# cbalint13/opencv-dlco

Measured on AMD Instinct MI355X. Metric: pj-learn patch-pairs/sec, higher is better.
Workload: dtype f32; 1 GPU; pj-learn configs[1] Liberty-shaped, rank ~64: 500000 pair-rows x PR-dim 8192, batch 200+200 per GPU (global 200+200), mu=0.0025 gamma=0.5, fp32, rank 48 after 3893 steps; device= (gfx950:sramecc+:xnack-), burn_in_steps=300

## Files before the change

opencv-dlco_amd/csrc/kernels_bf16x2.hip:

```cpp
#include "dlco_internal.hpp"
#include "split_bf16_dev.hpp"

#include <algorithm>

namespace dlco {

namespace {

constexpr int W8 = 8;
constexpr int T8 = 64 * W8;
constexpr int KS = 4;

__global__ __launch_bounds__(256) void split_x_kernel(const float *X, long ldx, int M, int MT, int K, bf16x8 *hi, bf16x8 *lo,
                                                      bf16x8 *lo2)
{
    const long t = (long)blockIdx.x * blockDim.x + threadIdx.x;
    const long total = (long)(K / 16) * MT * 64;
    if (t >= total) return;
    const int lane = (int)(t & 63);
    const long q = t >> 6;
    const int tile = (int)(q % MT);
    const int k16 = (int)(q / MT);
    const int row = tile * 32 + (lane & 31), k = k16 * 16 + 8 * (lane >> 5);
    bf16x8 h, l, l2;
    if (row < M) {
        const f32x4 a = *reinterpret_cast<const f32x4 *>(X + (long)row * ldx + k);
        const f32x4 b = *reinterpret_cast<const f32x4 *>(X + (long)row * ldx + k + 4);
#pragma unroll
        for (int j = 0; j < 8; j++) split_f32<3>(j < 4 ? a[j & 3] : b[j & 3], j, h, l, l2);
    } else {
        h = l = l2 = bf16x8{};
    }
    hi[t] = h;
    lo[t] = l;
    if (lo2) lo2[t] = l2;
}

struct Bf2Dev {
    int M, N, K;
    const bf16x8 *xhi, *xlo, *xlo2;
    const float *G;
    long ldg;
    float *slab;
    int tiled;
};

template <int MT, int NS>
__global__ __launch_bounds__(T8) void skinny_bf16x2_kernel(Bf2Dev g)
{
    __shared__ float red[4 * MT * 16 * 64];
    const int lane = threadIdx.x & 63, wave = threadIdx.x >> 6;
    const int lc = lane & 31, lh = lane >> 5;
    const int ct = wave & 3, kh = wave >> 2;
    const int col = blockIdx.x * 128 + ct * 32 + lc;
    const int nsteps = g.K / 16;
    const int per = nsteps / ((int)gridDim.y * 2);
    const int s0 = (blockIdx.y * 2 + kh) * per, s1 = s0 + per;

    f32x16 acc[MT];
#pragma unroll
    for (int a = 0; a < MT; a++)
#pragma unroll
        for (int r = 0; r < 16; r++) acc[a][r] = 0.f;

    bf16x8 ah[MT], al[MT], ahn[MT], aln[MT];
    bf16x8 am[NS == 3 ? MT : 1], amn[NS == 3 ? MT : 1];
    auto load_g = [&](int s, float (&gv)[8]) {
        const float *p = g.G + ((long)s * 16 + 8 * lh) * g.ldg + col;
#pragma unroll
        for (int j = 0; j < 8; j++) gv[j] = p[(long)j * g.ldg];
    };
    auto load_a = [&](int s, bf16x8 (&h)[MT], bf16x8 (&l)[MT], bf16x8 (&m2)[NS == 3 ? MT : 1]) {
#pragma unroll
        for (int t = 0; t < MT; t++) {
            const long idx = plane_entry((long)s, MT, t, lane);
            h[t] = g.xhi[idx];
            l[t] = g.xlo[idx];
            if (NS == 3) m2[t] = g.xlo2[idx];
        }
    };
    auto compute = [&](const float (&gv)[8], const bf16x8 (&h)[MT], const bf16x8 (&l)[MT], const bf16x8 (&m2)[NS == 3 ? MT : 1]) {
        bf16x8 bh, bl, bl2;
        split_frag<NS>(gv, bh, bl, bl2);
        mfma_split_terms<MT, NS>(h, l, m2, bh, bl, bl2, acc);
    };

    float gq[4][8];
    const int last = s1 - 1;
#pragma unroll
    for (int q = 0; q < 4; q++) load_g(s0 + q, gq[q]);
    load_a(s0, ah, al, am);
    load_a(s0 + 1, ahn, aln, amn);
    for (int s = s0; s < s1; s += 4) {
        compute(gq[0], ah, al, am);
        load_g(min(s + 4, last), gq[0]);
        load_a(min(s + 2, last), ah, al, am);
        compute(gq[1], ahn, aln, amn);
        load_g(min(s + 5, last), gq[1]);
        load_a(min(s + 3, last), ahn, aln, amn);
        compute(gq[2], ah, al, am);
        load_g(min(s + 6, last), gq[2]);
        load_a(min(s + 4, last), ah, al, am);
        compute(gq[3], ahn, aln, amn);
        load_g(min(s + 7, last), gq[3]);
        load_a(min(s + 5, last), ahn, aln, amn);
    }

    if (kh == 1) {
#pragma unroll
        for (int a = 0; a < MT; a++)
#pragma unroll
            for (int r = 0; r < 16; r++) red[((ct * MT + a) * 16 + r) * 64 + lane] = acc[a][r];
    }
    __syncthreads();
    if (kh == 0) {
        float *slab = g.slab + (long)blockIdx.y * g.M * g.N;
#pragma unroll
        for (int a = 0; a < MT; a++)
#pragma unroll
            for (int r = 0; r < 16; r++) {
                const float s = acc[a][r] + red[((ct * MT + a) * 16 + r) * 64 + lane];
                const int i = a * 32 + (r & 3) + 8 * (r >> 2) + 4 * lh;
                if (i < g.M) slab[(long)i * g.N + col] = s;
            }
    }
}


template <int MT, int NS>
__global__ __launch_bounds__(SB_T) void skinny_rows_kernel(Bf2Dev g)
{
    extern __shared__ __attribute__((aligned(16))) char lds_raw[];
    constexpr int ABYTES = sb_abytes(MT, NS);
    constexpr int APLANE = MT * 256;
    constexpr int NA = NS * MT;
    float *gb0 = reinterpret_cast<float *>(lds_raw), *gb1 = reinterpret_cast<float *>(lds_raw + SB_GBYTES);
    bf16x8 *ab0 = reinterpret_cast<bf16x8 *>(lds_raw + 2 * SB_GBYTES), *ab1 = reinterpret_cast<bf16x8 *>(lds_raw + 2 * SB_GBYTES + ABYTES);
    const int tid = threadIdx.x, lane = tid & 63, wave = tid >> 6;
    int bx = blockIdx.x, by = blockIdx.y;
    {
        const int gx = gridDim.x, ks = gridDim.y;
        if (ks <= 8 && 8 % ks == 0 && (gx * ks) % 8 == 0 && gx % (8 / ks) == 0) {
            const int b = by * gx + bx, xcd = b & 7, w = b >> 3, per = 8 / ks;
            by = xcd / per;
            bx = w * per + xcd % per;
        }
    }
    const int j0 = bx * 128;
    const int kslice = g.K / (int)gridDim.y;
    const int kbeg = by * kslice;
    const int nchunks = kslice / SB_KC;
    const int st0 = kbeg / 16;

    if (wave >= 8) {
        const int lt = tid - 512, grow = lt >> 4, gc4 = lt & 15;
        const __amdgpu_buffer_rsrc_t rsrc =
            __builtin_amdgcn_make_buffer_rsrc(const_cast<float *>(g.G), 0, (int)((long)g.K * g.ldg * (long)sizeof(float)), 0x00020000);
        const long pitch = g.tiled ? 128 : g.ldg;
        const long base = g.tiled ? ((long)bx * (g.K / 128) + kbeg / 128) * 16384 + (long)grow * 128 + 4 * gc4
                                  : (long)(j0 + grow) * g.ldg + kbeg + 4 * gc4;
        const int voff = (int)(base * (long)sizeof(float));
        const int row16 = (int)(16 * pitch * (long)sizeof(float));
        const PlaneRsrc rs = make_plane_rsrc<MT, NS>(g.xhi, g.xlo, g.xlo2, g.K);
        struct Stage { f32x4 gq[8]; bf16x8 aq[NA]; };
        Stage s0, s1;
        auto gload = [&](int c, Stage &st) {
            const int soff = g.tiled ? ((c >> 1) * 16384 + (c & 1) * 64) * (int)sizeof(float) : c * SB_KC * (int)sizeof(float);
#pragma unroll
            for (int u = 0; u < 8; u++) st.gq[u] = __builtin_bit_cast(f32x4, __builtin_amdgcn_raw_buffer_load_b128(rsrc, voff, soff + u * row16, 0));
            const int a0 = slice_bytes<MT>(st0 + 4 * c);
#pragma unroll
            for (int v = 0; v < NA; v++) st.aq[v] = load_slice_entry<MT>(rs, a0, lt, v);
        };
        auto gstore = [&](int buf, const Stage &st) {
            float *gb = buf ? gb1 : gb0;
            bf16x8 *ab = buf ? ab1 : ab0;
#pragma unroll
            for (int u = 0; u < 8; u++) *reinterpret_cast<f32x4 *>(gb + (grow + 16 * u) * SB_RS + 4 * gc4) = st.gq[u];
#pragma unroll
            for (int v = 0; v < NA; v++) ab[lt + 256 * v] = st.aq[v];
        };
        const int last = nchunks - 1;
        gload(0, s0);
        gload(min(1, last), s1);
        gstore(0, s0);
        gload(min(2, last), s0);
        __syncthreads();
        auto full = [&](int buf, Stage &set, int cc) { gstore(buf, set); gload(cc + 3, set); __syncthreads(); };
        auto part = [&](int buf, Stage &set, int cc) {
            if (cc >= nchunks) return;
            if (cc + 1 < nchunks) gstore(buf, set);
            if (cc + 3 < nchunks) gload(cc + 3, set);
            __syncthreads();
        };
        int c = 0;
        for (; c + 4 < nchunks; c += 2) { full(1, s1, c); full(0, s0, c + 1); }
        part(1, s1, c); part(0, s0, c + 1); part(1, s1, c + 2); part(0, s0, c + 3);
        __syncthreads();
        return;
    }

    const int lc = lane & 31, lh = lane >> 5;
    const int nt = wave & 3, kh = wave >> 2;
    f32x16 acc[MT];
#pragma unroll
    for (int a = 0; a < MT; a++)
#pragma unroll
        for (int r = 0; r < 16; r++) acc[a][r] = 0.f;

    auto fetch = [&](const float *gb, const bf16x8 *ab, int q, Frag<MT, NS> &f) {
        const float *p = gb + (nt * 32 + lc) * SB_RS + 16 * q + 8 * lh;
        f.g0 = *reinterpret_cast<const f32x4 *>(p);
        f.g1 = *reinterpret_cast<const f32x4 *>(p + 4);
#pragma unroll
        for (int n = 0; n < NS; n++)
#pragma unroll
            for (int t = 0; t < MT; t++) f.a[n][t] = ab[n * APLANE + plane_entry(q, MT, t, lane)];
    };
    auto multiply = [&](const Frag<MT, NS> &f) {
        bf16x8 bh, bl, bl2;
        split_frag<NS>(f.g0, f.g1, bh, bl, bl2);
        mfma_split_terms<MT, NS>(f.a[0], f.a[NS >= 2 ? 1 : 0], f.a[NS - 1], bh, bl, bl2, acc);
    };
    Frag<MT, NS> fa;
    __syncthreads();
    for (int c = 0; c < nchunks; c++) {
        const float *gb = (c & 1) ? gb1 : gb0;
        const bf16x8 *ab = (c & 1) ? ab1 : ab0;
        fetch(gb, ab, 2 * kh, fa);
        multiply(fa);
        fetch(gb, ab, 2 * kh + 1, fa);
        multiply(fa);
        __syncthreads();
    }

    float *red = reinterpret_cast<float *>(lds_raw);
    if (kh == 1) {
#pragma unroll
        for (int a = 0; a < MT; a++)
#pragma unroll
            for (int r = 0; r < 16; r++) red[((nt * MT + a) * 16 + r) * 64 + lane] = acc[a][r];
    }
    __syncthreads();
    if (kh == 0) {
        float *slab = g.slab + (long)by * g.M * g.N;
        const int col = j0 + nt * 32 + lc;
#pragma unroll
        for (int a = 0; a < MT; a++)
#pragma unroll
            for (int r = 0; r < 16; r++) {
                const float sum = acc[a][r] + red[((nt * MT + a) * 16 + r) * 64 + lane];
                const int i = a * 32 + (r & 3) + 8 * (r >> 2) + 4 * lh;
                if (i < g.M) slab[(long)i * g.N + col] = sum;
            }
    }
}

__global__ __launch_bounds__(256) void reduce_split_kernel(const float *slab, int split, int M, int MT, int N, float *C, long ldc, float alpha,
                                                           const float *E1, float b1, const float *E2, float b2, bf16x8 *hi, bf16x8 *lo)
{
    const long total = (long)M * N, q = N >> 3;
    for (long e = (long)blockIdx.x * blockDim.x + threadIdx.x; e < (long)M * q; e += (long)gridDim.x * blockDim.x) {
        const int i = (int)(e / q), k8 = (int)(e % q), j = k8 * 8;
        const float *p = slab + (long)i * N + j;
        f32x4 s0 = *reinterpret_cast<const f32x4 *>(p), s1 = *reinterpret_cast<const f32x4 *>(p + 4);
        for (int z = 1; z < split; z++) {
            s0 += *reinterpret_cast<const f32x4 *>(p + (long)z * total);
            s1 += *reinterpret_cast<const f32x4 *>(p + (long)z * total + 4);
        }
        const long idx = (long)i * ldc + j;
        f32x4 o0 = alpha * s0, o1 = alpha * s1;
        if (E1) { o0 += b1 * *reinterpret_cast<const f32x4 *>(E1 + idx); o1 += b1 * *reinterpret_cast<const f32x4 *>(E1 + idx + 4); }
        if (E2) { o0 += b2 * *reinterpret_cast<const f32x4 *>(E2 + idx); o1 += b2 * *reinterpret_cast<const f32x4 *>(E2 + idx + 4); }
        *reinterpret_cast<f32x4 *>(C + idx) = o0;
        *reinterpret_cast<f32x4 *>(C + idx + 4) = o1;
        bf16x8 h, l, l2;
        split_frag<2>(o0, o1, h, l, l2);
        const long t = plane_entry_at(MT, i, k8);
        hi[t] = h;
        lo[t] = l;
    }
}

constexpr int SYM_TS = 132;
static_assert(SB_KC * SYM_TS * 4 <= SB_GBYTES, "a transposed chunk image must fit the G image");

struct SymDev {
    int M, K;
    int nt, lb;
    const bf16x8 *xhi, *xlo, *xlo2;
    const float *G;
    float *slab;
};

template <int MT, int NS, bool FULL>
__global__ __launch_bounds__(SB_T) void skinny_sym_kernel(SymDev g)
{
    extern __shared__ __attribute__((aligned(16))) char lds_raw[];
    constexpr int ABYTES = sb_abytes(MT, NS);
    constexpr int APLANE = MT * 256;
    constexpr int NA = NS * MT;
    const int NT = g.nt, lb = g.lb;
    float *gb0 = reinterpret_cast<float *>(lds_raw), *gb1 = reinterpret_cast<float *>(lds_raw + SB_GBYTES);
    bf16x8 *ab0 = reinterpret_cast<bf16x8 *>(lds_raw + 2 * SB_GBYTES), *ab1 = reinterpret_cast<bf16x8 *>(lds_raw + 2 * SB_GBYTES + ABYTES);
    __shared__ int jlist[16];
    const int tid = threadIdx.x, lane = tid & 63, wave = tid >> 6;
    const int xcd = blockIdx.x & 7, slot = blockIdx.x >> 3;
    const int p = xcd >> 1, c = xcd & 1;
    int I;
    if (p == 0 || p == 3) I = (c << (lb - 1)) | slot;
    else {
        const int b5 = slot >> (lb - 2), b4 = p == 1 ? c : (b5 ^ c);
        I = (b5 << (lb - 1)) | (b4 << (lb - 2)) | (slot & ((1 << (lb - 2)) - 1));
    }
    if (I >= NT) return;
    const int dbase = (p == 0 ? 1 : (p == 1 ? 2 : (p == 2 ? 3 : 0))) << (lb - 2);
    int nchunks;
    if (FULL) nchunks = 2 << (lb - 2);
    else {
        const int nslots = 1 << (lb - 2);
        int cnt = 0;
        for (int sl = 0; sl < nslots; sl++) {
            const int J = I ^ (dbase | sl);
            if (J < NT) { if (tid == 0) jlist[cnt] = J; cnt++; }
        }
        nchunks = 2 * cnt;
        __syncthreads();
    }
    if (!FULL && nchunks == 0) {
        float *slab = g.slab + (long)p * g.M * g.K;
        for (int e = tid; e < g.M * 128; e += SB_T) slab[(long)(e >> 7) * g.K + I * 128 + (e & 127)] = 0.f;
        return;
    }
    auto partner = [&](int cc) { return FULL ? (I ^ (dbase | (cc >> 1))) : jlist[cc >> 1]; };
    auto tile_bytes = [&](int J) {
        const int a = min(I, J), b = max(I, J);
        return (a * NT - a * (a - 1) / 2 + (b - a)) * (128 * 128 * (int)sizeof(float));
    };

    if (wave >= 8) {
        const int lt = tid - 512;
        const int voff_d = ((lt >> 4) * 128 + 4 * (lt & 15)) * (int)sizeof(float);
        const int voff_t = ((lt >> 5) * 128 + 4 * (lt & 31)) * (int)sizeof(float);
        const int loff_d = (lt >> 4) * SB_RS + 4 * (lt & 15), loff_t = (lt >> 5) * SYM_TS + 4 * (lt & 31);
        const __amdgpu_buffer_rsrc_t rsrc =
            __builtin_amdgcn_make_buffer_rsrc(const_cast<float *>(g.G), 0, (NT * (NT + 1) / 2) * 128 * 128 * (int)sizeof(float), 0x00020000);
        const PlaneRsrc rs = make_plane_rsrc<MT, NS>(g.xhi, g.xlo, g.xlo2, g.K);
        struct Stage { f32x4 gq[8]; bf16x8 aq[NA]; };
        Stage s0, s1;
        auto gload = [&](int cc, Stage &st) {
            const int J = __builtin_amdgcn_readfirstlane(partner(cc)), half = cc & 1;
            const bool direct = I <= J;
            const int voff = direct ? voff_d : voff_t;
            const int soff = tile_bytes(J) + (direct ? half * 64 : half * 64 * 128) * (int)sizeof(float);
            const int ustep = (direct ? 16 : 8) * 128 * (int)sizeof(float);
            const int a0 = slice_bytes<MT>(J * 8 + half * 4);
            __builtin_amdgcn_sched_barrier(0);
#pragma unroll
            for (int u = 0; u < 8; u++) {
                st.gq[u] = __builtin_bit_cast(f32x4, __builtin_amdgcn_raw_buffer_load_b128(rsrc, voff, soff + u * ustep, 0));
                __builtin_amdgcn_sched_barrier(0);
            }
#pragma unroll
            for (int v = 0; v < NA; v++) {
                st.aq[v] = load_slice_entry<MT>(rs, a0, lt, v);
                __builtin_amdgcn_sched_barrier(0);
            }
        };
        auto gstore = [&](int cc, const Stage &st) {
            float *gb = (cc & 1) ? gb1 : gb0;
            bf16x8 *ab = (cc & 1) ? ab1 : ab0;
            const bool direct = I <= partner(cc);
            const int loff = direct ? loff_d : loff_t, lstep = direct ? 16 * SB_RS : 8 * SYM_TS;
#pragma unroll
            for (int u = 0; u < 8; u++) *reinterpret_cast<f32x4 *>(gb + loff + u * lstep) = st.gq[u];
#pragma unroll
            for (int v = 0; v < NA; v++) ab[lt + 256 * v] = st.aq[v];
        };
        gload(0, s0);
        gload(1, s1);
        gstore(0, s0);
        gload(min(2, nchunks - 1), s0);
        __syncthreads();
        int cc = 0;
        for (; cc + 4 < nchunks; cc += 2) {
            gstore(cc + 1, s1); gload(cc + 3, s1); __syncthreads();
            gstore(cc + 2, s0); gload(cc + 4, s0); __syncthreads();
        }
        for (; cc < nchunks; cc += 2) {
            if (cc + 1 < nchunks) gstore(cc + 1, s1);
            if (cc + 3 < nchunks) gload(cc + 3, s1);
            __syncthreads();
            if (cc + 2 < nchunks) gstore(cc + 2, s0);
            if (cc + 4 < nchunks) gload(cc + 4, s0);
            __syncthreads();
        }
        __syncthreads();
        return;
    }

    const int lc = lane & 31, lh = lane >> 5;
    const int nt = wave & 3, kh = wave >> 2;
    f32x16 acc[MT];
#pragma unroll
    for (int a = 0; a < MT; a++)
#pragma unroll
        for (int r = 0; r < 16; r++) acc[a][r] = 0.f;

    auto fetch = [&](const float *gb, const bf16x8 *ab, bool direct, int q, Frag<MT, NS> &f) {
        if (direct) {
            const float *pp = gb + (nt * 32 + lc) * SB_RS + 16 * q + 8 * lh;
            f.g0 = *reinterpret_cast<const f32x4 *>(pp);
            f.g1 = *reinterpret_cast<const f32x4 *>(pp + 4);
        } else {
            const float *pp = gb + (16 * q + 8 * lh) * SYM_TS + nt * 32 + lc;
#pragma unroll
            for (int j = 0; j < 4; j++) { f.g0[j] = pp[j * SYM_TS]; f.g1[j] = pp[(4 + j) * SYM_TS]; }
        }
#pragma unroll
        for (int n = 0; n < NS; n++)
#pragma unroll
            for (int t = 0; t < MT; t++) f.a[n][t] = ab[n * APLANE + plane_entry(q, MT, t, lane)];
    };
    auto multiply = [&](const Frag<MT, NS> &f) {
        bf16x8 bh, bl, bl2;
        split_frag<NS>(f.g0, f.g1, bh, bl, bl2);
        mfma_split_terms<MT, NS>(f.a[0], f.a[NS >= 2 ? 1 : 0], f.a[NS - 1], bh, bl, bl2, acc);
    };
    Frag<MT, NS> fa;
    __syncthreads();
    for (int cc = 0; cc < nchunks; cc++) {
        const float *gb = (cc & 1) ? gb1 : gb0;
        const bf16x8 *ab = (cc & 1) ? ab1 : ab0;
        const bool direct = I <= partner(cc);
        fetch(gb, ab, direct, 2 * kh, fa);
        multiply(fa);
        fetch(gb, ab, direct, 2 * kh + 1, fa);
        multiply(fa);
        __syncthreads();
    }

    float *red = reinterpret_cast<float *>(lds_raw);
    if (kh == 1) {
#pragma unroll
        for (int a = 0; a < MT; a++)
#pragma unroll
            for (int r = 0; r < 16; r++) red[((nt * MT + a) * 16 + r) * 64 + lane] = acc[a][r];
    }
    __syncthreads();
    if (kh == 0) {
        float *slab = g.slab + (long)p * g.M * g.K;
        const int col = I * 128 + nt * 32 + lc;
#pragma unroll
        for (int a = 0; a < MT; a++)
#pragma unroll
            for (int r = 0; r < 16; r++) {
                const float sum = acc[a][r] + red[((nt * MT + a) * 16 + r) * 64 + lane];
                const int i = a * 32 + (r & 3) + 8 * (r >> 2) + 4 * lh;
                if (i < g.M) slab[(long)i * g.K + col] = sum;
            }
    }
}

template <int MT, int NS>
void launch_sym(const SymDev &g, hipStream_t s)
{
    const size_t lds = sb_lds_bytes(MT, NS);
    if (g.nt == (1 << g.lb)) {
        ensure_dynamic_lds(reinterpret_cast<const void *>(skinny_sym_kernel<MT, NS, true>), (int)lds);
        hipLaunchKernelGGL((skinny_sym_kernel<MT, NS, true>), dim3(4u << g.lb), dim3(SB_T), lds, s, g);
    } else {
        ensure_dynamic_lds(reinterpret_cast<const void *>(skinny_sym_kernel<MT, NS, false>), (int)lds);
        hipLaunchKernelGGL((skinny_sym_kernel<MT, NS, false>), dim3(4u << g.lb), dim3(SB_T), lds, s, g);
    }
}

template <int MT, int NS>
void launch_rows(const Bf2Dev &g, dim3 grid, hipStream_t s)
{
    const size_t lds = sb_lds_bytes(MT, NS);
    ensure_dynamic_lds(reinterpret_cast<const void *>(skinny_rows_kernel<MT, NS>), (int)lds);
    hipLaunchKernelGGL((skinny_rows_kernel<MT, NS>), grid, dim3(SB_T), lds, s, g);
}

}

void split_planes_bf16(const float *X, long ldx, int M, int K, void *hi, void *lo, void *lo2, hipStream_t s)
{
    const int mt = (M + 31) / 32;
    const long total = (long)(K / 16) * mt * 64;
    hipLaunchKernelGGL(split_x_kernel, dim3((unsigned)((total + 255) / 256)), dim3(256), 0, s, X, ldx, M, mt, K,
                       static_cast<bf16x8 *>(hi), static_cast<bf16x8 *>(lo), static_cast<bf16x8 *>(lo2));
    DLCO_HIP(hipGetLastError());
}

size_t bf16x2_plane_bytes(int M, int K) { return (size_t)((M + 31) / 32) * 32 * K * sizeof(__bf16); }
size_t bf16x2_slab_floats(int M, int N, int ksplit) { return (size_t)(ksplit > 0 ? ksplit : KS) * M * N; }

bool skinny_product_bf16x2(const float *X, long ldx, int M, const float *G, long ldg, int N, int K, float alpha, float *C,
                           long ldc, const float *E1, float b1, const float *E2, float b2, void *plane_hi, void *plane_lo,
                           float *slab, hipStream_t s, int ksplit, void *plane_lo2, bool g_tiled)
{
    const int mt = (M + 31) / 32;
    const int ks = ksplit > 0 ? ksplit : KS;
    if (M < 1 || mt > 5 || N % 128 != 0 || K % (16 * ks * 2 * 4) != 0) return false;
    if (ldx % 4 != 0 || (reinterpret_cast<uintptr_t>(X) & 15) != 0) return false;
    split_planes_bf16(X, ldx, M, K, plane_hi, plane_lo, plane_lo2, s);
    Bf2Dev g;
    g.M = M; g.N = N; g.K = K;
    g.xhi = static_cast<const bf16x8 *>(plane_hi); g.xlo = static_cast<const bf16x8 *>(plane_lo);
    g.xlo2 = static_cast<const bf16x8 *>(plane_lo2);
    g.G = G; g.ldg = ldg; g.slab = slab; g.tiled = g_tiled ? 1 : 0;
    const dim3 grid(N / 128, ks), block(T8);
    if (N == K && K % (128 * ks) == 0 && ldg % 4 == 0 && (reinterpret_cast<uintptr_t>(G) & 15) == 0 &&
        (long)K * ldg * 4 < (1L << 31) && !(mt >= 4 && plane_lo2)) {
        if (plane_lo2) dispatch_mt<4>(mt, [&](auto MT) { launch_rows<MT(), 3>(g, grid, s); });
        else dispatch_mt<5>(mt, [&](auto MT) { launch_rows<MT(), 2>(g, grid, s); });
        DLCO_HIP(hipGetLastError());
        splitk_reduce_f32(slab, ks, M, N, C, ldc, alpha, 0.f, E1, b1, E2, b2, s);
        return true;
    }
    if (g_tiled || mt > 4) return false;
    if (plane_lo2) dispatch_mt<4>(mt, [&](auto MT) { hipLaunchKernelGGL((skinny_bf16x2_kernel<MT(), 3>), grid, block, 0, s, g); });
    else dispatch_mt<4>(mt, [&](auto MT) { hipLaunchKernelGGL((skinny_bf16x2_kernel<MT(), 2>), grid, block, 0, s, g); });
    DLCO_HIP(hipGetLastError());
    splitk_reduce_f32(slab, ks, M, N, C, ldc, alpha, 0.f, E1, b1, E2, b2, s);
    return true;
}

bool skinny_product_sym(const float *X, long ldx, int M, const float *Gpacked, int F, float alpha, float *C, long ldc,
                        const float *E1, float b1, const float *E2, float b2, void *plane_hi, void *plane_lo, float *slab,
                        hipStream_t s, void *plane_lo2, bool planes_ready, bool emit_planes)
{
    const int mt = (M + 31) / 32;
    const int nt = F / 128;
    if (F % 128 != 0 || nt < 1 || nt > 64 || M < 1 || mt > 5 || (mt >= 4 && plane_lo2)) return false;
    if (ldx % 4 != 0 || (reinterpret_cast<uintptr_t>(X) & 15) != 0 || (reinterpret_cast<uintptr_t>(Gpacked) & 15) != 0) return false;
    if ((planes_ready || emit_planes) && plane_lo2) return false;
    if (!planes_ready) split_planes_bf16(X, ldx, M, F, plane_hi, plane_lo, plane_lo2, s);
    SymDev g;
    g.M = M; g.K = F;
    g.nt = nt; g.lb = 2;
    while ((1 << g.lb) < nt) g.lb++;
    g.xhi = static_cast<const bf16x8 *>(plane_hi); g.xlo = static_cast<const bf16x8 *>(plane_lo); g.xlo2 = static_cast<const bf16x8 *>(plane_lo2);
    g.G = Gpacked; g.slab = slab;
    if (plane_lo2) dispatch_mt<3>(mt, [&](auto MT) { launch_sym<MT(), 3>(g, s); });
    else dispatch_mt<5>(mt, [&](auto MT) { launch_sym<MT(), 2>(g, s); });
    DLCO_HIP(hipGetLastError());
    if (emit_planes && ldc % 4 == 0 && (reinterpret_cast<uintptr_t>(C) & 15) == 0) {
        const long work = (long)M * (F / 8);
        hipLaunchKernelGGL(reduce_split_kernel, dim3((unsigned)std::min<long>((work + 255) / 256, 4096)), dim3(256), 0, s, slab, 4, M, mt, F, C, ldc,
                           alpha, E1, b1, E2, b2, static_cast<bf16x8 *>(plane_hi), static_cast<bf16x8 *>(plane_lo));
        DLCO_HIP(hipGetLastError());
    } else {
        splitk_reduce_f32(slab, 4, M, F, C, ldc, alpha, 0.f, E1, b1, E2, b2, s);
    }
    return true;
}

}
```

Measured before the change: 710,900 pair-rows/s.

## Stream symmetric-kernel operands into a four-stage LDS ring via direct global-to-LDS loads

Replaces the producer waves' register-staged double buffer in the symmetric skinny GEMM with a four-stage LDS ring. Producers fill it with global_load_lds (buffer loads go straight into LDS) and pace themselves with explicit vmcnt waits and barriers. Consumers now use a software-pipelined loop that fetches and converts the next stage while running MFMAs on the current one, and the tile and plane layouts are re-indexed to match the new LDS image. The goal is to cut the register round-trip and LDS store work on the producers and to hide load latency, at the cost of more LDS use and fragile hand-counted waits and barriers.

```diff
diff --git a/opencv-dlco_amd/csrc/kernels_bf16x2.hip b/opencv-dlco_amd/csrc/kernels_bf16x2.hip
--- a/opencv-dlco_amd/csrc/kernels_bf16x2.hip
+++ b/opencv-dlco_amd/csrc/kernels_bf16x2.hip
@@ -2,6 +2,7 @@
 #include "split_bf16_dev.hpp"
 
 #include <algorithm>
+#include <type_traits>
 
 namespace dlco {
 
@@ -282,8 +283,20 @@
     }
 }
 
-constexpr int SYM_TS = 132;
-static_assert(SB_KC * SYM_TS * 4 <= SB_GBYTES, "a transposed chunk image must fit the G image");
+constexpr int SYM_NSTAGE = 4;
+constexpr int SYM_GBYTES = SB_ROWS * (SB_KC / 2) * 4;
+__host__ __device__ constexpr int sym_abytes(int mt, int ns) { return 2 * ns * mt * 1024; }
+__host__ __device__ constexpr int sym_stage_bytes(int mt, int ns) { return SYM_GBYTES + sym_abytes(mt, ns); }
+inline size_t sym_lds_bytes(int mt, int ns) { return (size_t)SYM_NSTAGE * sym_stage_bytes(mt, ns); }
+#ifndef SYM_PREFETCH
+#define SYM_PREFETCH 1
+#endif
+#ifndef SYM_PREFETCH_MAX
+#define SYM_PREFETCH_MAX 9
+#endif
+constexpr int SYM_LDS_MAX = 160 * 1024 - 64;
+static_assert(SYM_NSTAGE * sym_stage_bytes(5, 2) <= SYM_LDS_MAX && SYM_NSTAGE * sym_stage_bytes(3, 3) <= SYM_LDS_MAX,
+              "the ring of the largest instantiations (five row tiles two-way, three three-way) must fit the LDS");
 
 struct SymDev {
     int M, K;
@@ -293,16 +306,24 @@
     float *slab;
 };
 
+template <int N>
+__device__ __forceinline__ void wait_vmcnt()
+{
+    asm volatile("s_waitcnt vmcnt(%0)" ::"n"(N) : "memory");
+}
+
 template <int MT, int NS, bool FULL>
 __global__ __launch_bounds__(SB_T) void skinny_sym_kernel(SymDev g)
 {
     extern __shared__ __attribute__((aligned(16))) char lds_raw[];
-    constexpr int ABYTES = sb_abytes(MT, NS);
-    constexpr int APLANE = MT * 256;
-    constexpr int NA = NS * MT;
+    constexpr int STAGE = sym_stage_bytes(MT, NS);
+    constexpr int NAP = 2 * NS * MT;
+    constexpr int NPIECE = 16 + NAP;
+    constexpr int PW = (NPIECE + 3) / 4;
+    constexpr bool PF = SYM_PREFETCH && MT * NS <= SYM_PREFETCH_MAX;
+    static_assert(3 * PW <= 63, "the in-flight count must fit the vmcnt field");
+    static_assert(4 * MT * 16 * 64 * 4 <= SYM_NSTAGE * STAGE, "the K-half exchange reuses the ring");
     const int NT = g.nt, lb = g.lb;
-    float *gb0 = reinterpret_cast<float *>(lds_raw), *gb1 = reinterpret_cast<float *>(lds_raw + SB_GBYTES);
-    bf16x8 *ab0 = reinterpret_cast<bf16x8 *>(lds_raw + 2 * SB_GBYTES), *ab1 = reinterpret_cast<bf16x8 *>(lds_raw + 2 * SB_GBYTES + ABYTES);
     __shared__ int jlist[16];
     const int tid = threadIdx.x, lane = tid & 63, wave = tid >> 6;
     const int xcd = blockIdx.x & 7, slot = blockIdx.x >> 3;
@@ -315,87 +336,92 @@
     }
     if (I >= NT) return;
     const int dbase = (p == 0 ? 1 : (p == 1 ? 2 : (p == 2 ? 3 : 0))) << (lb - 2);
-    int nchunks;
-    if (FULL) nchunks = 2 << (lb - 2);
+    int nst;
+    unsigned jmask = 0;
+    if (FULL) nst = 4 << (lb - 2);
     else {
         const int nslots = 1 << (lb - 2);
         int cnt = 0;
         for (int sl = 0; sl < nslots; sl++) {
             const int J = I ^ (dbase | sl);
-            if (J < NT) { if (tid == 0) jlist[cnt] = J; cnt++; }
-        }
-        nchunks = 2 * cnt;
+            if (J < NT) { if (tid == 0) jlist[cnt] = J; cnt++; jmask |= 1u << sl; }
+        }
+        nst = 4 * cnt;
         __syncthreads();
     }
-    if (!FULL && nchunks == 0) {
+    if (!FULL && nst == 0) {
         float *slab = g.slab + (long)p * g.M * g.K;
         for (int e = tid; e < g.M * 128; e += SB_T) slab[(long)(e >> 7) * g.K + I * 128 + (e & 127)] = 0.f;
         return;
     }
-    auto partner = [&](int cc) { return FULL ? (I ^ (dbase | (cc >> 1))) : jlist[cc >> 1]; };
     auto tile_bytes = [&](int J) {
         const int a = min(I, J), b = max(I, J);
         return (a * NT - a * (a - 1) / 2 + (b - a)) * (128 * 128 * (int)sizeof(float));
     };
 
     if (wave >= 8) {
-        const int lt = tid - 512;
-        const int voff_d = ((lt >> 4) * 128 + 4 * (lt & 15)) * (int)sizeof(float);
-        const int voff_t = ((lt >> 5) * 128 + 4 * (lt & 31)) * (int)sizeof(float);
-        const int loff_d = (lt >> 4) * SB_RS + 4 * (lt & 15), loff_t = (lt >> 5) * SYM_TS + 4 * (lt & 31);
-        const __amdgpu_buffer_rsrc_t rsrc =
-            __builtin_amdgcn_make_buffer_rsrc(const_cast<float *>(g.G), 0, (NT * (NT + 1) / 2) * 128 * 128 * (int)sizeof(float), 0x00020000);
-        const PlaneRsrc rs = make_plane_rsrc<MT, NS>(g.xhi, g.xlo, g.xlo2, g.K);
-        struct Stage { f32x4 gq[8]; bf16x8 aq[NA]; };
-        Stage s0, s1;
-        auto gload = [&](int cc, Stage &st) {
-            const int J = __builtin_amdgcn_readfirstlane(partner(cc)), half = cc & 1;
+        const int lw = __builtin_amdgcn_readfirstlane(wave - 8);
+        const char *Gb = reinterpret_cast<const char *>(g.G);
+        const int off_d = (lane & 15) * 512 + (lane >> 4) * 16;
+        const int off_t0 = (lane >> 5) * 512 + (lane & 31) * 16, off_t1 = (lane >> 5) * 512 + ((lane & 31) ^ 8) * 16;
+        const char *asrc[PW - 4];
+        int adst[PW - 4];
+#pragma unroll
+        for (int i = 4; i < PW; i++) {
+            const int a = min(lw + 4 * i - 16, NAP - 1);
+            const int akh = a / (NS * MT), part = (a / MT) % NS, t = a % MT;
+            const bf16x8 *plane = part == 0 ? g.xhi : (part == 1 ? g.xlo : g.xlo2);
+            asrc[i - 4] = reinterpret_cast<const char *>(plane) + (2 * akh * MT + t) * 1024 + lane * 16;
+            adst[i - 4] = SYM_GBYTES + a * 1024;
+        }
+        int J = 0;
+        auto issue = [&](int st) {
+            if ((st & 3) == 0) {
+                if (FULL) J = I ^ (dbase | (st >> 2));
+                else {
+                    J = I ^ (dbase | (__builtin_ctz(jmask)));
+                    jmask &= jmask - 1;
+                }
+                J = __builtin_amdgcn_readfirstlane(J);
+            }
+            const int half = (st >> 1) & 1, h = st & 1;
             const bool direct = I <= J;
-            const int voff = direct ? voff_d : voff_t;
-            const int soff = tile_bytes(J) + (direct ? half * 64 : half * 64 * 128) * (int)sizeof(float);
-            const int ustep = (direct ? 16 : 8) * 128 * (int)sizeof(float);
-            const int a0 = slice_bytes<MT>(J * 8 + half * 4);
-            __builtin_amdgcn_sched_barrier(0);
-#pragma unroll
-            for (int u = 0; u < 8; u++) {
-                st.gq[u] = __builtin_bit_cast(f32x4, __builtin_amdgcn_raw_buffer_load_b128(rsrc, voff, soff + u * ustep, 0));
-                __builtin_amdgcn_sched_barrier(0);
+            const char *tile = Gb + tile_bytes(J);
+            char *dst = lds_raw + (st & (SYM_NSTAGE - 1)) * STAGE;
+#pragma unroll
+            for (int i = 0; i < 4; i++) {
+                const int pc = lw + 4 * i;
+                const int od = ((pc >> 1) * 16) * 512 + half * 256 + (2 * (pc & 1) + h) * 64;
+                const int ot = (half * 64 + (2 * (i >> 1) + h) * 16 + 2 * lw + 8 * (i & 1)) * 512;
+                const int off = direct ? od + off_d : ot + ((i & 1) ? off_t1 : off_t0);
+                __builtin_amdgcn_global_load_lds((const __attribute__((address_space(1))) void *)(tile + off),
+                                                 (__attribute__((address_space(3))) void *)(dst + pc * 1024), 16, 0, 0);
             }
-#pragma unroll
-            for (int v = 0; v < NA; v++) {
-                st.aq[v] = load_slice_entry<MT>(rs, a0, lt, v);
-                __builtin_amdgcn_sched_barrier(0);
-            }
+            const int a_off = (J * 8 + half * 4 + h) * MT * 1024;
+#pragma unroll
+            for (int i = 4; i < PW; i++)
+                __builtin_amdgcn_global_load_lds((const __attribute__((address_space(1))) void *)(asrc[i - 4] + a_off),
+                                                 (__attribute__((address_space(3))) void *)(dst + adst[i - 4]), 16, 0, 0);
         };
-        auto gstore = [&](int cc, const Stage &st) {
-            float *gb = (cc & 1) ? gb1 : gb0;
-            bf16x8 *ab = (cc & 1) ? ab1 : ab0;
-            const bool direct = I <= partner(cc);
-            const int loff = direct ? loff_d : loff_t, lstep = direct ? 16 * SB_RS : 8 * SYM_TS;
-#pragma unroll
-            for (int u = 0; u < 8; u++) *reinterpret_cast<f32x4 *>(gb + loff + u * lstep) = st.gq[u];
-#pragma unroll
-            for (int v = 0; v < NA; v++) ab[lt + 256 * v] = st.aq[v];
-        };
-        gload(0, s0);
-        gload(1, s1);
-        gstore(0, s0);
-        gload(min(2, nchunks - 1), s0);
-        __syncthreads();
-        int cc = 0;
-        for (; cc + 4 < nchunks; cc += 2) {
-            gstore(cc + 1, s1); gload(cc + 3, s1); __syncthreads();
-            gstore(cc + 2, s0); gload(cc + 4, s0); __syncthreads();
-        }
-        for (; cc < nchunks; cc += 2) {
-            if (cc + 1 < nchunks) gstore(cc + 1, s1);
-            if (cc + 3 < nchunks) gload(cc + 3, s1);
-            __syncthreads();
-            if (cc + 2 < nchunks) gstore(cc + 2, s0);
-            if (cc + 4 < nchunks) gload(cc + 4, s0);
-            __syncthreads();
-        }
-        __syncthreads();
+        issue(0); issue(1); issue(2);
+        if (PF) {
+            issue(3);
+            wait_vmcnt<3 * PW>();
+            __builtin_amdgcn_s_barrier();
+        }
+        for (int st = 0; st + 3 + PF < nst; st++) {
+            wait_vmcnt<2 * PW>();
+            __builtin_amdgcn_s_barrier();
+            issue(st + 3 + PF);
+        }
+        wait_vmcnt<2 * PW>();
+        __builtin_amdgcn_s_barrier();
+        wait_vmcnt<PW>();
+        __builtin_amdgcn_s_barrier();
+        wait_vmcnt<0>();
+        __builtin_amdgcn_s_barrier();
+        __builtin_amdgcn_s_barrier();
+        __builtin_amdgcn_s_barrier();
         return;
     }
 
@@ -407,20 +433,24 @@
 #pragma unroll
         for (int r = 0; r < 16; r++) acc[a][r] = 0.f;
 
-    auto fetch = [&](const float *gb, const bf16x8 *ab, bool direct, int q, Frag<MT, NS> &f) {
+    auto partner = [&](int sl) { return FULL ? (I ^ (dbase | sl)) : jlist[sl]; };
+    const int n = nt * 32 + lc;
+    const int rd_d = (((n >> 4) * 8 + kh * 4 + lh * 2) * 16 + (n & 15)) * 16;
+    const int rd_t = ((kh * 16 + lh * 8) * 128 + (n ^ (32 * lh))) * 4;
+    auto fetch = [&](const char *sb, bool direct, Frag<MT, NS> &f) {
         if (direct) {
-            const float *pp = gb + (nt * 32 + lc) * SB_RS + 16 * q + 8 * lh;
-            f.g0 = *reinterpret_cast<const f32x4 *>(pp);
-            f.g1 = *reinterpret_cast<const f32x4 *>(pp + 4);
+            f.g0 = *reinterpret_cast<const f32x4 *>(sb + rd_d);
+            f.g1 = *reinterpret_cast<const f32x4 *>(sb + rd_d + 256);
         } else {
-            const float *pp = gb + (16 * q + 8 * lh) * SYM_TS + nt * 32 + lc;
-#pragma unroll
-            for (int j = 0; j < 4; j++) { f.g0[j] = pp[j * SYM_TS]; f.g1[j] = pp[(4 + j) * SYM_TS]; }
-        }
-#pragma unroll
-        for (int n = 0; n < NS; n++)
-#pragma unroll
-            for (int t = 0; t < MT; t++) f.a[n][t] = ab[n * APLANE + plane_entry(q, MT, t, lane)];
+            const float *pp = reinterpret_cast<const float *>(sb + rd_t);
+#pragma unroll
+            for (int j = 0; j < 4; j++) { f.g0[j] = pp[j * 128]; f.g1[j] = pp[(4 + j) * 128]; }
+        }
+        const bf16x8 *ab = reinterpret_cast<const bf16x8 *>(sb + SYM_GBYTES);
+#pragma unroll
+        for (int s = 0; s < NS; s++)
+#pragma unroll
+            for (int t = 0; t < MT; t++) f.a[s][t] = ab[((kh * NS + s) * MT + t) * 64 + lane];
     };
     auto multiply = [&](const Frag<MT, NS> &f) {
         bf16x8 bh, bl, bl2;
@@ -428,19 +458,56 @@
         mfma_split_terms<MT, NS>(f.a[0], f.a[NS >= 2 ? 1 : 0], f.a[NS - 1], bh, bl, bl2, acc);
     };
     Frag<MT, NS> fa;
-    __syncthreads();
-    for (int cc = 0; cc < nchunks; cc++) {
-        const float *gb = (cc & 1) ? gb1 : gb0;
-        const bf16x8 *ab = (cc & 1) ? ab1 : ab0;
-        const bool direct = I <= partner(cc);
-        fetch(gb, ab, direct, 2 * kh, fa);
-        multiply(fa);
-        fetch(gb, ab, direct, 2 * kh + 1, fa);
-        multiply(fa);
-        __syncthreads();
-    }
-
     float *red = reinterpret_cast<float *>(lds_raw);
+    auto stage_barrier = [&] {
+        __builtin_amdgcn_sched_barrier(0);
+        asm volatile("s_waitcnt lgkmcnt(0)" ::: "memory");
+        __builtin_amdgcn_s_barrier();
+        asm volatile("" ::: "memory");
+        __builtin_amdgcn_sched_barrier(0);
+    };
+    auto stage_ptr = [&](int st) { return lds_raw + (st & (SYM_NSTAGE - 1)) * STAGE; };
+    if constexpr (PF) {
+        struct BFrag { bf16x8 h, l, l2; };
+        auto convert = [&](const Frag<MT, NS> &f, BFrag &b) {
+            split_frag<NS>(f.g0, f.g1, b.h, b.l, b.l2);
+            if (NS == 3) asm volatile("" : "+v"(b.h), "+v"(b.l), "+v"(b.l2));
+            else asm volatile("" : "+v"(b.h), "+v"(b.l));
+        };
+        auto mfmas = [&](const Frag<MT, NS> &f, const BFrag &b) {
+            mfma_split_terms<MT, NS>(f.a[0], f.a[NS >= 2 ? 1 : 0], f.a[NS - 1], b.h, b.l, b.l2, acc);
+        };
+        Frag<MT, NS> fb;
+        BFrag ba, bb;
+        stage_barrier();
+        fetch(stage_ptr(0), I <= partner(0), fa);
+        convert(fa, ba);
+        auto trip = [&](int st, auto more) {
+            stage_barrier();
+            fetch(stage_ptr(st + 1), I <= partner((st + 1) >> 2), fb);
+            __builtin_amdgcn_sched_barrier(0);
+            mfmas(fa, ba);
+            __builtin_amdgcn_sched_barrier(0);
+            convert(fb, bb);
+            stage_barrier();
+            if constexpr (decltype(more)::value) fetch(stage_ptr(st + 2), I <= partner((st + 2) >> 2), fa);
+            __builtin_amdgcn_sched_barrier(0);
+            mfmas(fb, bb);
+            __builtin_amdgcn_sched_barrier(0);
+            if constexpr (decltype(more)::value) convert(fa, ba);
+        };
+        int st = 0;
+        for (; st + 2 < nst; st += 2) trip(st, std::true_type{});
+        trip(st, std::false_type{});
+    } else {
+        for (int st = 0; st < nst; st++) {
+            stage_barrier();
+            fetch(stage_ptr(st), I <= partner(st >> 2), fa);
+            multiply(fa);
+        }
+        stage_barrier();
+    }
+
     if (kh == 1) {
 #pragma unroll
         for (int a = 0; a < MT; a++)
@@ -465,7 +532,7 @@
 template <int MT, int NS>
 void launch_sym(const SymDev &g, hipStream_t s)
 {
-    const size_t lds = sb_lds_bytes(MT, NS);
+    const size_t lds = sym_lds_bytes(MT, NS);
     if (g.nt == (1 << g.lb)) {
         ensure_dynamic_lds(reinterpret_cast<const void *>(skinny_sym_kernel<MT, NS, true>), (int)lds);
         hipLaunchKernelGGL((skinny_sym_kernel<MT, NS, true>), dim3(4u << g.lb), dim3(SB_T), lds, s, g);
```

Result: slower. 691,000 pair-rows/s (-2.8%).
